# dflaxx/3d-hashjoin

Measured on AMD Instinct MI355X. Metric: probe tuples/s + build ms, exp1 key/FK |R|=1e7 |S|=1e8, 1/2/4/8 GPU, higher is better.
Workload: dtype u32; 1 GPU; exp1 key/FK plan Csr, |R|=10000000 |S|=100000000 per GPU, uniform FKs, b=1; config=B, plan=Csr, R_total=10000000, S_total=100000000, R_per_gpu=10000000, S_per_gpu=100000000, num_buckets=10000000, emit_pairs=True, parallelism=single GPU, rehearsal_one_gpu=False

## Files before the change

3d-hashjoin_amd/csrc/chain_pk.hip:

```cpp
#include <cmath>

#include "radix_seg.hpp"

namespace hj3d {
namespace {

constexpr int kPkBlock = 1024;
constexpr int kPkRounds = 8;
constexpr int kPkTile = kPkBlock * kPkRounds;
constexpr int kPkTBits = 32 - __builtin_clz(uint32_t(kPkTile - 1));
constexpr uint32_t kPkSeg = 16;
constexpr uint32_t kPkStage2 = 15872;
static_assert(kPkTile <= kPkStage2 && kPkStage2 < 65536, "the tile alone fits the stage; stage offsets in 16 bits");
constexpr uint32_t kPkMaxP1 = 2 * kPkBlock;
constexpr uint32_t kSortedMaxPk = 32;
constexpr uint32_t kOvfFlag = 0x80000000u;

enum { kCtlNovf = 0, kCtlOut = 1, kCtlTicket = 2, kCtlOvfCursor = 3, kCtlNprobe = 4, kCtlWords = 8 };


__device__ __forceinline__ void pk_ovf_append(bool me, uint2 e, uint2* __restrict__ ovf, uint64_t* ctl) {
  const uint64_t m = __ballot(me);
  if (!m) return;
  const int lane = threadIdx.x & 63;
  const int leader = __ffsll((unsigned long long)m) - 1;
  uint64_t b = 0;
  if (lane == leader) b = atomicAdd(reinterpret_cast<unsigned long long*>(ctl + kCtlNovf), (unsigned long long)__popcll(m));
  b = __shfl(b, leader, kWave);
  const uint64_t lt = lane == 0 ? 0ull : (~0ull >> (64 - lane));
  if (me) ovf[b + __popcll(m & lt)] = e;
}

template <int PPT>
struct PkPartGeom {
  static constexpr uint32_t kSeg = kPkSeg / PPT;
  static constexpr uint32_t kStage = kPkStage2;
};
template <bool IMPLICIT, bool SEL, int PPT>
__device__ __forceinline__ void pk_part_stage(const RelView& r, const PkGeom& pk, uint32_t ntiles, uint32_t cap,
                                              uint2* __restrict__ region, uint32_t* __restrict__ counts,
                                              uint2* __restrict__ ovf, uint64_t* __restrict__ ctl,
                                              const SelRange& sel, uint32_t stage_lim) {
  constexpr uint32_t SEG = PkPartGeom<PPT>::kSeg, STAGE = PkPartGeom<PPT>::kStage;
  __shared__ uint2 stage[STAGE];
  __shared__ uint32_t loc[kPkBlock * PPT];
  __shared__ uint32_t sbase[kPkBlock * PPT];
  __shared__ uint2 seginfo[STAGE / SEG];
  __shared__ uint32_t wsum[kPkBlock / kWave];
  const uint32_t me = threadIdx.x, P = pk.P, n = uint32_t(r.n);
  const int lane = threadIdx.x & 63, wid = threadIdx.x >> 6;
  const auto sl = [&](int k) __attribute__((always_inline)) { return me + uint32_t(k) * kPkBlock; };
  uint32_t my_reg[PPT];
  uint2 creg[PPT][SEG - 1];
  uint32_t my_kc[PPT], my_cur[PPT], my_end[PPT];
#pragma unroll
  for (int k = 0; k < PPT; ++k) {
    my_reg[k] = (blockIdx.x * P + sl(k)) * cap;
    my_kc[k] = 0;
    my_cur[k] = 0;
    my_end[k] = cap;
#pragma unroll
    for (int j = 0; j < int(SEG) - 1; ++j) creg[k][j] = make_uint2(0, 0);
  }
  uint32_t ha[kPkRounds], pa[SEL ? kPkRounds : 1];
  uint32_t wa[IMPLICIT ? 1 : kPkRounds];
  auto load = [&](uint32_t (&h)[kPkRounds], uint32_t (&pw)[SEL ? kPkRounds : 1],
                  uint32_t (&rw)[IMPLICIT ? 1 : kPkRounds], uint32_t tile) __attribute__((always_inline)) {
    const uint32_t base = tile * kPkTile;
#pragma unroll
    for (int j = 0; j < kPkRounds; ++j) {
      const uint32_t i = base + uint32_t(j) * kPkBlock + me;
      const char* t = r.base + uint64_t(i) * r.stride;
      h[j] = i < n ? __builtin_nontemporal_load(reinterpret_cast<const uint32_t*>(t + r.key_off)) : 0u;
      if constexpr (!IMPLICIT)
        rw[j] = i < n ? __builtin_nontemporal_load(reinterpret_cast<const uint32_t*>(t + r.row_off)) : 0u;
      if constexpr (SEL) pw[j] = i < n ? *reinterpret_cast<const uint32_t*>(t + sel.word_off) : 0u;
    }
  };
  auto to_ovf = [&](uint2 e, uint32_t p, bool me_) __attribute__((always_inline)) {
    pk_ovf_append(me_, make_uint2(pk.hash_of(e.x, p), e.y), ovf, ctl);
  };
  auto flush_carry = [&]() __attribute__((always_inline)) {
#pragma unroll
    for (int k = 0; k < PPT; ++k) {
#pragma unroll
      for (int j = 0; j < int(SEG) - 1; ++j) {
        const bool v = sl(k) < P && uint32_t(j) < my_kc[k];
        const uint32_t o = my_cur[k] + j;
        if (v && o < my_end[k]) region[my_reg[k] + o] = creg[k][j];
        to_ovf(creg[k][j], sl(k), v && o >= my_end[k]);
      }
      my_cur[k] += my_kc[k];
      my_kc[k] = 0;
    }
  };
  auto scan = [&](uint32_t v, uint32_t* total) __attribute__((always_inline)) {
    uint32_t x = v;
#pragma unroll
    for (int o = 1; o < 64; o <<= 1) {
      const uint32_t y = __shfl_up(x, o, kWave);
      if (lane >= o) x += y;
    }
    if (lane == 63) wsum[wid] = x;
    __syncthreads();
    uint32_t pre = 0, tot = 0;
#pragma unroll
    for (int w = 0; w < kPkBlock / kWave; ++w) {
      const uint32_t t = wsum[w];
      if (w < wid) pre += t;
      tot += t;
    }
    __syncthreads();
    *total = tot;
    return pre + x - v;
  };
  uint32_t npassed = 0;
  auto process = [&](uint32_t tile, uint32_t (&h)[kPkRounds], uint32_t (&pw)[SEL ? kPkRounds : 1],
                     uint32_t (&rw)[IMPLICIT ? 1 : kPkRounds]) __attribute__((always_inline)) {
    const uint32_t base = tile * kPkTile;
    uint32_t rk[kPkRounds];
#pragma unroll
    for (int j = 0; j < kPkRounds; ++j) {
      const uint32_t i = base + uint32_t(j) * kPkBlock + me;
      const uint32_t hv = murmur32(h[j]);
      const uint32_t q = pk.dnb.div(hv);
      const uint32_t bl = hv - q * pk.nb - pk.lo;
      bool pass = i < n;
      if constexpr (SEL) {
        pass = pass && sel.test(pw[j]);
        npassed += pass;
      }
      const bool ok = pass && bl < pk.nbl;
      rk[j] = kInvalid;
      if (ok) {
        const uint32_t p = pk.dw.div(bl);
        h[j] = ((bl - p * pk.W) << pk.qbits) | q;
        rk[j] = (p << kPkTBits) | atomicAdd(&loc[p], 1u);
      }
    }
    __syncthreads();
    uint32_t my_c[PPT];
#pragma unroll
    for (int k = 0; k < PPT; ++k) {
      my_c[k] = sl(k) < P ? loc[sl(k)] : 0u;
      loc[sl(k)] = 0;
    }
    const auto seg_counts = [&](int k) __attribute__((always_inline)) {
      const uint32_t L = my_kc[k] + my_c[k];
      return (L << 16) | (L / SEG);
    };
    const auto seg_sum = [&]() __attribute__((always_inline)) {
      uint32_t t = 0;
#pragma unroll
      for (int k = 0; k < PPT; ++k) t += seg_counts(k);
      return t;
// ... 404 lines not shown
                                               const uint32_t* ldir, const uint2* lent, const PkGeom& pk,
                                               uint64_t (&acc)[kProbeFields], uint2* __restrict__ out,
                                               uint64_t out_cap) {
  uint32_t nm = 0, sc = 0, nv = 0;
  constexpr int H = (K == 8 || (CK && K == 7)) ? (K + 1) / 2 : K;
#pragma unroll
  for (int g = 0; g < K; g += H) {
    uint32_t d[H], match[H], cmps[H], q[H];
    bool live[H];
#pragma unroll
    for (int j = 0; j < H && g + j < K; ++j) {
      const bool ok = (valid >> (g + j)) & 1u;
      const uint32_t x = uint32_t(v[g + j]);
      q[j] = x & pk.qmask;
      const uint32_t w = ldir[ok ? x >> pk.qbits : 0u];
      d[j] = ok ? w : 0u;
      match[j] = kInvalid;
      cmps[j] = d[j] & 0xFFFFu;
      live[j] = cmps[j] != 0 && cmps[j] <= kSortedMaxPk;
    }
#pragma unroll
    for (uint32_t c = 0; c < 3; ++c) {
      uint64_t e[H];
      bool ok[H];
#pragma unroll
      for (int j = 0; j < H && g + j < K; ++j) {
        const uint32_t nn = d[j] & 0xFFFFu;
        ok[j] = live[j] && c < nn;
        e[j] = *reinterpret_cast<const uint64_t*>(lent + (ok[j] ? (d[j] >> 16) + (c == 0 ? 0u : nn - c) : 0u));
      }
#pragma unroll
      for (int j = 0; j < H && g + j < K; ++j) asm volatile("" : "+v"(e[j]));
#pragma unroll
      for (int j = 0; j < H && g + j < K; ++j) {
        const bool hit = ok[j] && uint32_t(e[j]) == q[j];
        match[j] = hit ? uint32_t(e[j] >> 32) : match[j];
        cmps[j] = hit ? c + 1 : cmps[j];
        live[j] = live[j] && !hit;
      }
    }
#pragma unroll
    for (int j = 0; j < H && g + j < K; ++j) {
      const uint32_t nn = d[j] & 0xFFFFu, s = d[j] >> 16;
      if (live[j] && nn > 3) {
        for (uint32_t c = 3; c < nn; ++c) {
          const uint2 e = lent[s + nn - c];
          if (e.x == q[j]) {
            cmps[j] = c + 1;
            match[j] = e.y;
            break;
          }
        }
      } else if (nn > kSortedMaxPk) {
        uint32_t minrow = kInvalid, lo_m = kInvalid, hi_m = 0, cnt = 0;
        for (uint32_t k = s; k < s + nn; ++k) {
          const uint2 e = lent[k];
          minrow = min(minrow, e.y);
          if (e.x == q[j]) {
            ++cnt;
            lo_m = min(lo_m, e.y);
            hi_m = max(hi_m, e.y);
          }
        }
        if (cnt != 0 && lo_m == minrow) {
          cmps[j] = 1;
          match[j] = lo_m;
        } else if (cnt != 0) {
          uint32_t gt = 0;
          for (uint32_t k = s; k < s + nn; ++k) gt += lent[k].y > hi_m;
          cmps[j] = 2 + gt;
          match[j] = hi_m;
        }
      }
    }
#pragma unroll
    for (int j = 0; j < H && g + j < K; ++j) {
      const bool ok = (valid >> (g + j)) & 1u;
      const uint32_t row = uint32_t(v[g + j] >> 32);
      const bool m = match[j] != kInvalid;
      nv += ok;
      nm += m;
      sc += cmps[j];
      if (MODE == 1) {
        const uint64_t slot = slot0 + uint32_t((g + j) * 64);
        if (ok && slot < out_cap) pair_st(out + slot, row, match[j]);
      }
      if (CK && m) {
        acc[4] += row;
        acc[5] += match[j];
        const uint64_t ph = pair_hash(row, match[j]);
        acc[7] += ph;
        acc[8] ^= ph;
      }
    }
  }
  acc[1] += nm;
  acc[2] += nm;
  acc[3] += sc;
  (void)nv;
}

template <int MODE, bool CK>
__device__ __forceinline__ void pk_probe_hbm(uint32_t h, uint32_t row, uint32_t s, uint32_t nn,
                                             const uint2* __restrict__ ent, uint64_t slot,
                                             uint64_t (&acc)[kProbeFields], uint2* __restrict__ out,
                                             uint64_t out_cap) {
  uint32_t match = kInvalid, cmps = nn;
  if (nn <= kSortedMaxPk) {
    for (uint32_t c = 0; c < nn; ++c) {
      const uint2 e = ent[s + (c == 0 ? 0u : nn - c)];
      if (e.x == h) {
        cmps = c + 1;
        match = e.y;
        break;
      }
    }
  } else {
    uint32_t minrow = kInvalid, lo_m = kInvalid, hi_m = 0, cnt = 0;
    for (uint32_t k = s; k < s + nn; ++k) {
      const uint2 e = ent[k];
      minrow = min(minrow, e.y);
      if (e.x == h) {
        ++cnt;
        lo_m = min(lo_m, e.y);
        hi_m = max(hi_m, e.y);
      }
    }
    if (cnt != 0 && lo_m == minrow) {
      cmps = 1;
      match = lo_m;
    } else if (cnt != 0) {
      uint32_t gt = 0;
      for (uint32_t k = s; k < s + nn; ++k) gt += ent[k].y > hi_m;
      cmps = 2 + gt;
      match = hi_m;
    }
  }
  acc[3] += cmps;
  if (match != kInvalid) {
    acc[1] += 1;
    acc[2] += 1;
    if (CK) {
      acc[4] += row;
      acc[5] += match;
      const uint64_t ph = pair_hash(row, match);
      acc[7] += ph;
      acc[8] ^= ph;
    }
  }
  if (MODE == 1 && slot < out_cap)
    __builtin_nontemporal_store((uint64_t(match) << 32) | row, reinterpret_cast<uint64_t*>(out + slot));
}

__device__ __forceinline__ void pk_stage(const uint32_t* __restrict__ off, const uint2* __restrict__ ent, uint32_t b0,
                                         uint32_t nbs, uint32_t e0, uint32_t ne, const FastDiv32& dnb, uint32_t* ldir,
                                         uint2* lent) {
  constexpr int kStage = 12;
  const uint32_t nmax = max(nbs, ne);
  for (uint32_t k0 = threadIdx.x; k0 < nmax; k0 += kPkBlock * kStage) {
    uint32_t a[kStage], b[kStage];
    uint2 x[kStage];
#pragma unroll
    for (int u = 0; u < kStage; ++u) {
      const uint32_t k = k0 + u * kPkBlock;
      a[u] = k < nbs ? off[b0 + k] : 0u;
      b[u] = k < nbs ? off[b0 + k + 1] : 0u;
      x[u] = k < ne ? ent[e0 + k] : make_uint2(0, 0);
    }
#pragma unroll
    for (int u = 0; u < kStage; ++u) {
      const uint32_t k = k0 + u * kPkBlock;
      if (k < nbs) ldir[k] = ((a[u] - e0) << 16) | (b[u] - a[u]);
      if (k < ne) lent[k] = make_uint2(dnb.div(x[u].x), x[u].y);
    }
  }
}

template <int K, int MODE, bool CK>
__global__ __launch_bounds__(kPkBlock) void k_pk_probe(const uint2* __restrict__ region,
                                                       const uint32_t* __restrict__ counts, uint32_t G, uint32_t cap,
                                                       uint32_t splits, bool flat, const uint32_t* __restrict__ off,
                                                       const uint2* __restrict__ ent, PkGeom pk, FastMod fm,
                                                       uint2* __restrict__ out, uint64_t out_cap,
                                                       const uint2* __restrict__ ovf, uint64_t* __restrict__ ctl,
                                                       uint64_t* __restrict__ partials, uint64_t* __restrict__ res,
                                                       int accumulate) {
  constexpr int BLOCK = kPkBlock;
  __shared__ uint32_t lds[kLdsWords];
  __shared__ uint32_t wtot[BLOCK / kWave];
  __shared__ uint32_t rpre[BLOCK / kWave][65];
  __shared__ uint64_t bbase;
  __shared__ uint64_t red[BLOCK / kWave][kProbeFields];
  __shared__ uint32_t flag;
  const int lane = threadIdx.x & 63, wid = threadIdx.x >> 6;
  constexpr int kWaves = BLOCK / kWave;
  const uint32_t P = pk.P;
  const uint32_t p = blockIdx.x / splits, sp = blockIdx.x % splits;
  const uint32_t b0 = p * pk.W;
  const uint32_t nbs = min(pk.W, pk.nbl - b0);
  const uint32_t e0 = off[b0], e1 = off[b0 + nbs], ne = e1 - e0;
  const bool fits = (nbs + 2) + 2ull * ne <= kLdsWords;
  uint32_t* ldir = lds;
  uint2* lent = reinterpret_cast<uint2*>(lds + ((nbs + 2) & ~1u));
  uint64_t acc[kProbeFields] = {0, 0, 0, 0, 0, 0, 0, 0, 0};

  const uint32_t g_lo = uint32_t(uint64_t(G) * sp / splits), g_hi = uint32_t(uint64_t(G) * (sp + 1) / splits);
  const uint32_t nr = g_hi > g_lo + wid ? (g_hi - g_lo - wid + kWaves - 1) / kWaves : 0u;
  uint32_t my_len = 0;
  if (uint32_t(lane) < nr) my_len = counts[(g_lo + wid + kWaves * lane) * P + p];
  uint32_t wtotal;
  const uint32_t my_pre = wave_excl_scan(my_len, &wtotal);
  if (lane == 0) wtot[wid] = wtotal;
  rpre[wid][lane] = uint32_t(lane) < nr ? my_pre : ~0u;
  if (lane == 0) rpre[wid][64] = ~0u;
  __syncthreads();
  if (threadIdx.x == 0) {
    uint32_t t = 0;
    for (int w = 0; w < kWaves; ++w) t += wtot[w];
    bbase = (MODE == 1 && t) ? atomicAdd(reinterpret_cast<unsigned long long*>(ctl + kCtlOut), (unsigned long long)t) : 0ull;
  }
  uint32_t wpre = 0;
  for (int w = 0; w < wid; ++w) wpre += wtot[w];
  auto pre_at = [&](uint32_t k) __attribute__((always_inline)) { return uint32_t(__builtin_amdgcn_readlane(int(my_pre), int(k))); };
  auto len_at = [&](uint32_t k) __attribute__((always_inline)) { return uint32_t(__builtin_amdgcn_readlane(int(my_len), int(k))); };
  auto src_of = [&](uint32_t k) __attribute__((always_inline)) { return region + (g_lo + wid + kWaves * k) * P * cap + p * cap; };

  const auto src_off = [&](uint32_t k) __attribute__((always_inline)) {
    return int64_t((uint64_t(g_lo + wid + kWaves * k) * P + p) * cap);
  };
  uint32_t cr = 0, nst = rpre[wid][1];
  int64_t cbase = src_off(0);
  auto load_flat = [&](uint64_t (&v)[K], uint32_t f0) __attribute__((always_inline)) {
#pragma unroll
    for (int j = 0; j < K; ++j) {
      const uint32_t f = min(f0 + j * 64 + lane, wtotal - 1);
      while (f >= nst) {
        ++cr;
        cbase = src_off(cr) - int64_t(nst);
        nst = rpre[wid][cr + 1];
      }
      v[j] = pair_ld(region + (cbase + int64_t(f)));
    }
  };
  uint32_t r = 0, qq = 0, len = nr ? len_at(0) : 0u;
  while (r < nr && len == 0) {
    ++r;
    len = r < nr ? len_at(r) : 0u;
  }
  auto load_reg = [&](uint64_t (&v)[K], uint32_t rr, uint32_t q0, uint32_t ll) __attribute__((always_inline)) {
    const uint2* src = rr < nr ? src_of(rr) : region;
    const uint32_t last = ll ? ll - 1 : 0u;
#pragma unroll
    for (int j = 0; j < K; ++j)
      v[j] = pair_ld(src + min(q0 + j * 64 + lane, last));
  };
  auto probe_hbm_chunk = [&](const uint64_t (&v)[K], uint32_t valid, uint64_t slot0) __attribute__((always_inline)) {
#pragma unroll
    for (int j = 0; j < K; ++j) {
      if (!((valid >> j) & 1u)) continue;
      const uint32_t x = uint32_t(v[j]), bl = b0 + (x >> pk.qbits);
      const uint32_t s = off[bl];
      pk_probe_hbm<MODE, CK>(pk.hash_of(x, p), uint32_t(v[j] >> 32), s, off[bl + 1] - s, ent, slot0 + j * 64, acc,
                             out, out_cap);
    }
  };
  auto walk = [&](auto&& stage, auto&& probe) __attribute__((always_inline)) {
    constexpr uint32_t kChunk = 64 * K;
    uint64_t cur[K];
    if (flat) {
      if (wtotal) load_flat(cur, 0);
      stage();
      __syncthreads();
      if (wtotal == 0) return;
      for (uint32_t f0 = 0; f0 < wtotal; f0 += kChunk) {
        uint64_t nxt[K];
        load_flat(nxt, min(f0 + kChunk, (wtotal - 1) / kChunk * kChunk));
        uint32_t vm = 0;
#pragma unroll
        for (int j = 0; j < K; ++j) vm |= uint32_t(f0 + j * 64 + lane < wtotal) << j;
        probe(cur, vm, f0 + lane);
#pragma unroll
        for (int j = 0; j < K; ++j) cur[j] = nxt[j];
      }
    } else {
      load_reg(cur, r, qq, len);
      stage();
      __syncthreads();
      while (r < nr) {
        uint32_t nr_ = r, nq = qq + kChunk, nl = len;
        while (nr_ < nr && nq >= nl) {
          ++nr_;
          nq = 0;
          nl = nr_ < nr ? len_at(nr_) : 0u;
        }
        uint64_t nxt[K];
        load_reg(nxt, nr_, nq, nl);
        uint32_t vm = 0;
#pragma unroll
        for (int j = 0; j < K; ++j) vm |= uint32_t(qq + j * 64 + lane < len) << j;
        probe(cur, vm, pre_at(r) + qq + lane);
        r = nr_;
        qq = nq;
        len = nl;
#pragma unroll
        for (int j = 0; j < K; ++j) cur[j] = nxt[j];
      }
    }
  };
  if (fits) {
    walk([&]() __attribute__((always_inline)) { pk_stage(off, ent, b0, nbs, e0, ne, pk.dnb, ldir, lent); },
         [&](const uint64_t (&v)[K], uint32_t valid, uint32_t srel) __attribute__((always_inline)) {
           pk_probe_items<K, MODE, CK>(v, valid, bbase + wpre + srel, ldir, lent, pk, acc, out, out_cap);
         });
  } else {
    walk([&]() __attribute__((always_inline)) {},
         [&](const uint64_t (&v)[K], uint32_t valid, uint32_t srel) __attribute__((always_inline)) {
           probe_hbm_chunk(v, valid, bbase + wpre + srel);
         });
  }
  const uint64_t novf = __hip_atomic_load(ctl + kCtlNovf, __ATOMIC_RELAXED, __HIP_MEMORY_SCOPE_AGENT);
  if (novf) {
    for (;;) {
      __syncthreads();
      if (threadIdx.x == 0) {
        const uint64_t c = atomicAdd(reinterpret_cast<unsigned long long*>(ctl + kCtlOvfCursor), (unsigned long long)BLOCK);
        const uint64_t take = c < novf ? min(uint64_t(BLOCK), novf - c) : 0ull;
        bbase = c;
        flag = uint32_t(take);
        if (MODE == 1 && take)
          red[0][0] = atomicAdd(reinterpret_cast<unsigned long long*>(ctl + kCtlOut), (unsigned long long)take);
      }
      __syncthreads();
      const uint32_t take = flag;
      if (!take) break;
      const uint64_t c = bbase, ob = MODE == 1 ? red[0][0] : 0ull;
      if (threadIdx.x < take) {
        const uint2 e = ovf[c + threadIdx.x];
        const uint32_t bl = fm.mod(e.x) - pk.lo;
        const uint32_t s = off[bl];
        pk_probe_hbm<MODE, CK>(e.x, e.y, s, off[bl + 1] - s, ent, ob + threadIdx.x, acc, out, out_cap);
      }
    }
  }
  __syncthreads();
#pragma unroll
  for (int f = 1; f < kProbeFields; ++f) {
    const uint64_t w = f == kProbeFields - 1 ? wave_xor(acc[f]) : wave_sum(acc[f]);
    if (lane == 0) red[wid][f] = w;
  }
  __syncthreads();
  if (threadIdx.x < kProbeFields) {
    const int f = threadIdx.x;
    uint64_t a = 0;
    for (int w = 0; w < kWaves; ++w) a = f == kProbeFields - 1 ? (a ^ red[w][f]) : (a + red[w][f]);
    __hip_atomic_store(partials + uint64_t(blockIdx.x) * kProbeFields + f, f == 0 ? 0ull : a, __ATOMIC_RELAXED,
                       __HIP_MEMORY_SCOPE_AGENT);
  }
  if (wid == 0) {
    asm volatile("s_waitcnt vmcnt(0)" ::: "memory");
    if (threadIdx.x == 0) {
      const uint64_t t = __hip_atomic_fetch_add(ctl + kCtlTicket, 1ull, __ATOMIC_RELAXED, __HIP_MEMORY_SCOPE_AGENT);
      flag = t == gridDim.x - 1;
    }
  }
  __syncthreads();
  if (!flag) return;
  uint64_t sum[kProbeFields] = {0, 0, 0, 0, 0, 0, 0, 0, 0};
  for (uint32_t b = threadIdx.x; b < gridDim.x; b += BLOCK) {
#pragma unroll
    for (int f = 1; f < kProbeFields; ++f) {
      const uint64_t x = __hip_atomic_load(partials + uint64_t(b) * kProbeFields + f, __ATOMIC_RELAXED,
                                           __HIP_MEMORY_SCOPE_AGENT);
      sum[f] = f == kProbeFields - 1 ? (sum[f] ^ x) : (sum[f] + x);
    }
  }
  __syncthreads();
#pragma unroll
  for (int f = 1; f < kProbeFields; ++f) {
    const uint64_t w = f == kProbeFields - 1 ? wave_xor(sum[f]) : wave_sum(sum[f]);
    if (lane == 0) red[wid][f] = w;
  }
  __syncthreads();
  if (threadIdx.x < kProbeFields) {
    const int f = threadIdx.x;
    uint64_t a = 0;
    if (f == 0) {
      a = __hip_atomic_load(ctl + kCtlNprobe, __ATOMIC_RELAXED, __HIP_MEMORY_SCOPE_AGENT);
    } else {
      for (int w = 0; w < kWaves; ++w) a = f == kProbeFields - 1 ? (a ^ red[w][f]) : (a + red[w][f]);
    }
    if (accumulate) a = f == kProbeFields - 1 ? (res[f] ^ a) : (res[f] + a);
    res[f] = a;
  }
  if (!accumulate && threadIdx.x >= kProbeFields && threadIdx.x < 16) res[threadIdx.x] = 0;
  if (threadIdx.x < kCtlWords) __hip_atomic_store(ctl + threadIdx.x, 0ull, __ATOMIC_RELAXED, __HIP_MEMORY_SCOPE_AGENT);
}

constexpr uint32_t kPbW = 8192;
constexpr int kPbPer = 11;
constexpr uint32_t kPbStage = 12288;
static_assert(kPbPer * kPkBlock <= int(kPbStage), "a register-held slice fits the stage");

__global__ __launch_bounds__(256) void k_pk_slice_sums(const uint32_t* __restrict__ cnt2, uint32_t S2, uint32_t P,
                                                       uint32_t* __restrict__ tot) {
  const uint32_t p = blockIdx.x * 256 + threadIdx.x;
  if (p >= P) return;
  uint32_t t = 0;
  for (uint32_t s = 0; s < S2; ++s) t += cnt2[uint64_t(s) * P + p];
  tot[p] = t;
}

__device__ __forceinline__ void pb_lds_scan(uint32_t* a, uint32_t n, uint32_t* wsum) {
  constexpr int kPer = (kPbW + kPkBlock) / kPkBlock;
  const uint32_t t0 = threadIdx.x * kPer;
  uint32_t v[kPer], loc = 0;
#pragma unroll
  for (int k = 0; k < kPer; ++k) {
    v[k] = t0 + k < n ? a[t0 + k] : 0u;
    loc += v[k];
  }
  const int lane = threadIdx.x & 63, wid = threadIdx.x >> 6;
  uint32_t wt;
  const uint32_t pre = wave_excl_scan(loc, &wt);
  if (lane == 0) wsum[wid] = wt;
  __syncthreads();
  uint32_t base = 0;
  for (int w = 0; w < wid; ++w) base += wsum[w];
  uint32_t run = base + pre;
#pragma unroll
  for (int k = 0; k < kPer; ++k) {
    if (t0 + k < n) a[t0 + k] = run;
    run += v[k];
  }
  __syncthreads();
}

__global__ __launch_bounds__(kPkBlock) void k_pk_build(const uint2* __restrict__ fine, const uint32_t* __restrict__ cnt2,
                                                       uint32_t S2, uint32_t cap2, const uint32_t* __restrict__ ps,
                                                       PkGeom pk, uint32_t* __restrict__ off, uint2* __restrict__ ent) {
  __shared__ uint32_t cnt[kPbW + 1];
  __shared__ uint2 stage[kPbStage];
  __shared__ uint32_t wsum[kPkBlock / kWave];
  constexpr uint32_t kCap = kPbPer * kPkBlock;
  const uint32_t P = pk.P, nbl = pk.nbl, W = pk.W;
  auto gather = [&](uint32_t p, uint32_t i) __attribute__((always_inline)) {
    uint32_t run = 0;
    int64_t d = int64_t(uint64_t(p) * cap2);
    for (uint32_t sg = 0; sg < S2; ++sg) {
      if (i >= run) d = int64_t((uint64_t(sg) * P + p) * cap2) - int64_t(run);
      run += cnt2[uint64_t(sg) * P + p];
    }
    return fine[int64_t(i) + d];
  };
  const int lane = threadIdx.x & 63, wid = threadIdx.x >> 6;
  auto fits = [&](uint32_t p) __attribute__((always_inline)) {
    bool ok = true;
    for (uint32_t sg = 0; sg < S2; ++sg) ok = ok && cnt2[uint64_t(sg) * P + p] <= uint32_t(kPbPer) * 64u;
    return ok;
  };
  uint2 ea[kPbPer], eb[kPbPer];
  auto load = [&](uint2 (&e)[kPbPer], uint32_t p) __attribute__((always_inline)) {
    if (p >= P || !fits(p)) return;
    const uint32_t c = uint32_t(wid) < S2 ? cnt2[uint64_t(wid) * P + p] : 0u;
    const uint2* src = fine + (uint64_t(wid) * P + p) * cap2;
#pragma unroll
    for (int u = 0; u < kPbPer; ++u) {
      const uint32_t i = uint32_t(u) * 64u + lane;
      e[u] = i < c ? src[i] : make_uint2(0, 0);
    }
  };
  auto build = [&](uint2 (&e)[kPbPer], uint32_t p) __attribute__((always_inline)) {
    const uint32_t b0 = p * W;
    const uint32_t nbs = min(W, nbl - b0);
    const uint32_t s0 = ps[p], m = ps[p + 1] - s0;
    for (uint32_t k = threadIdx.x; k < nbs; k += kPkBlock) cnt[k] = 0;
    __syncthreads();
    if (!fits(p) || m > kCap) {
      for (uint32_t i = threadIdx.x; i < m; i += kPkBlock) atomicAdd(&cnt[gather(p, i).x >> pk.qbits], 1u);
      __syncthreads();
      pb_lds_scan(cnt, nbs, wsum);
      for (uint32_t k = threadIdx.x; k < nbs; k += kPkBlock) off[b0 + k] = s0 + cnt[k];
      if (b0 + nbs == nbl && threadIdx.x == 0) off[nbl] = s0 + m;
      __syncthreads();
      for (uint32_t i = threadIdx.x; i < m; i += kPkBlock) {
        const uint2 x = gather(p, i);
        ent[s0 + atomicAdd(&cnt[x.x >> pk.qbits], 1u)] = make_uint2(pk.hash_of(x.x, p), x.y);
      }
      __syncthreads();
      for (uint32_t k = threadIdx.x; k < nbs; k += kPkBlock) {
        const uint32_t bs = k ? cnt[k - 1] : 0u, n = cnt[k] - bs;
        if (n < 2 || n > kSortedMaxPk) continue;
        uint2* E = ent + s0 + bs;
        for (uint32_t q = 1; q < n; ++q) {
          const uint2 x = E[q];
          uint32_t j = q;
          while (j > 0 && E[j - 1].y > x.y) {
            E[j] = E[j - 1];
            --j;
          }
          E[j] = x;
        }
      }
      __syncthreads();
      return;
    }
    uint32_t rk[kPbPer];
    const uint32_t c = uint32_t(wid) < S2 ? cnt2[uint64_t(wid) * P + p] : 0u;
#pragma unroll
    for (int u = 0; u < kPbPer; ++u) {
      const bool v = uint32_t(u) * 64u + lane < c;
      const uint32_t b = v ? e[u].x >> pk.qbits : 0u;
      rk[u] = v ? (b << 16) | atomicAdd(&cnt[b], 1u) : kInvalid;
    }
    __syncthreads();
    pb_lds_scan(cnt, nbs, wsum);
    if (threadIdx.x == 0) cnt[nbs] = m;
    for (uint32_t k = threadIdx.x; k < nbs; k += kPkBlock) off[b0 + k] = s0 + cnt[k];
    if (b0 + nbs == nbl && threadIdx.x == 0) off[nbl] = s0 + m;
    __syncthreads();
#pragma unroll
    for (int u = 0; u < kPbPer; ++u)
      if (rk[u] != kInvalid) stage[cnt[rk[u] >> 16] + (rk[u] & 0xFFFFu)] = e[u];
    __syncthreads();
    for (uint32_t q = threadIdx.x; q < m; q += kPkBlock) {
      const uint2 x = stage[q];
      const uint32_t b = x.x >> pk.qbits;
      const uint32_t bs = cnt[b], n = cnt[b + 1] - bs;
      uint32_t pos = q;
      if (n >= 2 && n <= kSortedMaxPk) {
        uint32_t rr = 0;
        for (uint32_t k = bs; k < bs + n; ++k) rr += stage[k].y < x.y;
        pos = bs + rr;
      }
      ent[s0 + pos] = make_uint2(pk.hash_of(x.x, p), x.y);
    }
    __syncthreads();
  };
  load(ea, blockIdx.x);
  for (uint32_t p = blockIdx.x; p < P; p += 2 * gridDim.x) {
    load(eb, p + gridDim.x);
    build(ea, p);
    if (p + gridDim.x >= P) break;
    load(ea, p + 2 * gridDim.x);
    build(eb, p + gridDim.x);
  }
}

}

static int pk_items(double L) {
  int best = kItemsMax;
  double best_slots = 0.0;
  const double sd = std::sqrt(L > 1.0 ? L : 1.0);
  for (int K = kItemsMax; K >= kItemsMin; --K) {
    const double c = 64.0 * K;
    double slots = 0.0, wsum = 0.0;
    for (int z = -40; z <= 40; ++z) {
      const double x = L + 0.1 * z * sd, w = std::exp(-0.005 * z * z);
      slots += w * std::ceil((x < 1.0 ? 1.0 : x) / c) * c;
      wsum += w;
    }
    slots /= wsum;
    if (K == kItemsMax || slots < best_slots * 0.999) {
      best = K;
      best_slots = slots;
    }
  }
  return best;
}

bool pk_probe_applicable(const hj3d_ctx* ctx, const hj3d_table* t, uint64_t n_probe, uint32_t flags) {
  return t->desc.kind == HJ3D_CHAIN && (flags & HJ3D_PROBE_UNIQUE) && !ctx->force_direct && !ctx->pk_off &&
         n_probe >= ctx->radix_min && n_probe > 0 && t->nb_local >= 64 && t->desc.num_buckets >= 2 &&
         n_probe < (1ull << 32) && t->built;
}

static uint32_t pk_slice_width(double fill) {
  double W = double(kPkLdsWords) / (1.0 + 2.0 * fill);
  for (int i = 0; i < 6; ++i) W = (double(kPkLdsWords) - 2.0 - 12.0 * std::sqrt(W * fill)) / (1.0 + 2.0 * fill);
  return W < 64.0 ? 64u : uint32_t(W);
}

PkPlan pk_plan(const hj3d_ctx* ctx, uint32_t nbl, uint64_t n_build) {
  PkPlan pl;
  const double fill = n_build ? double(n_build) / double(nbl) : 0.0;
  uint32_t W = pk_slice_width(fill);
  if (ctx->pk_slice_max && W > ctx->pk_slice_max) W = ctx->pk_slice_max;
  if (W > nbl) W = nbl;
  uint32_t P = (nbl + W - 1) / W;
  const uint32_t ncu = uint32_t(ctx->num_cus);
  if (P >= ncu / 2) {
    uint32_t Pq = (P + ncu - 1) / ncu * ncu;
    if (P <= kPkMaxP1 && Pq > kPkMaxP1) Pq = kPkMaxP1;
    P = Pq;
    W = (nbl + P - 1) / P;
    P = (nbl + W - 1) / W;
  }
  pl.W = W;
  pl.P = P;
  pl.C = P <= kPkMaxP1 ? 1u : (P + kPkBlock - 1) / kPkBlock;
  pl.W1 = W * pl.C;
  pl.P1 = (nbl + pl.W1 - 1) / pl.W1;
  return pl;
}

static uint32_t bits(uint64_t x) {
  uint32_t b = 0;
  while (x) {
    ++b;
    x >>= 1;
  }
  return b;
}

struct PkLayout {
  uint32_t qbits = 0, ntiles = 0, G = 0, S2 = 0;
  uint64_t cap = 0, cap2 = 0, nreg = 0, nreg2 = 0;
  PkGeom pk1{}, pk{};
  uint2 *region = nullptr, *ovf = nullptr, *fine = nullptr;
  uint32_t *counts = nullptr, *fcnt = nullptr, *ps = nullptr;
  uint64_t* ctl = nullptr;
};

static hipError_t pk_layout(hj3d_ctx* ctx, const hj3d_table* t, uint64_t n, uint32_t W, uint32_t P, uint32_t C, bool two,
                            bool sums, PkLayout* L) {
  hipError_t e;
  const uint32_t nbl = t->nb_local, nb = uint32_t(t->desc.num_buckets);
  const uint32_t W1 = W * C, P1 = (nbl + W1 - 1) / W1;
  const uint32_t qbits = L->qbits = bits(0xFFFFFFFFull / nb);
  if (qbits + bits(W1 - 1) > 32) return hipErrorNotSupported;
  const uint32_t ntiles = L->ntiles = uint32_t((n + kPkTile - 1) / kPkTile);
  const uint32_t G = L->G = ntiles < uint32_t(ctx->num_cus) ? ntiles : uint32_t(ctx->num_cus);
  const uint64_t per_g = uint64_t((ntiles + G - 1) / G) * kPkTile;
  const uint64_t cap = L->cap = region_capacity(double(per_g < n ? per_g : n) / P1, kPkSeg);
  const uint64_t nreg = L->nreg = uint64_t(G) * P1;
  if (nreg * cap >= (1ull << 31)) return hipErrorNotSupported;
  const uint32_t S2 = L->S2 = two ? (G < 16u ? G : 16u) : 0u;
  const double per_gp = double(per_g < n ? per_g : n) / P;
  const uint64_t cap2 = L->cap2 = two ? region_capacity(per_gp * double((G + S2 - 1) / S2), kPkSeg) : 0;
  const uint64_t nreg2 = L->nreg2 = uint64_t(S2) * P;
  if (two && nreg2 * cap2 >= (1ull << 31)) return hipErrorNotSupported;
  if ((e = ctx->scratch[kScrPairs].ensure(nreg * cap * sizeof(uint2))) != hipSuccess) return e;
  if ((e = ctx->scratch[kScrPHist].ensure(nreg * sizeof(uint32_t))) != hipSuccess) return e;
  if ((e = ctx->scratch[kScrSortV].ensure(n * sizeof(uint2))) != hipSuccess) return e;
  if (two) {
    if ((e = ctx->scratch[kScrPk2].ensure(nreg2 * cap2 * sizeof(uint2))) != hipSuccess) return e;
    if ((e = ctx->scratch[kScrPk2Cnt].ensure(nreg2 * sizeof(uint32_t))) != hipSuccess) return e;
  }
  if (sums && (e = ctx->scratch[kScrPStart].ensure((uint64_t(P) + 1) * sizeof(uint32_t))) != hipSuccess) return e;
  if ((e = ctx->ensure_ctl()) != hipSuccess) return e;
  auto geom = [&](uint32_t w, uint32_t p) {
    PkGeom g;
    g.dnb = FastDiv32::make(nb);
    g.dw = w >= 2 ? FastDiv32::make(w) : FastDiv32{};
    g.nb = nb;
    g.lo = uint32_t(t->desc.bucket_lo);
    g.nbl = nbl;
    g.W = w;
    g.P = p;
    g.qbits = qbits;
    g.qmask = qbits >= 32 ? 0xFFFFFFFFu : ((1u << qbits) - 1);
    return g;
  };
  L->pk1 = geom(W1, P1);
  L->pk = geom(W, P);
  L->region = ctx->scratch[kScrPairs].as<uint2>();
  L->counts = ctx->scratch[kScrPHist].as<uint32_t>();
  L->ovf = ctx->scratch[kScrSortV].as<uint2>();
  L->fine = two ? ctx->scratch[kScrPk2].as<uint2>() : nullptr;
  L->fcnt = two ? ctx->scratch[kScrPk2Cnt].as<uint32_t>() : nullptr;
  L->ps = sums ? ctx->scratch[kScrPStart].as<uint32_t>() : nullptr;
  L->ctl = ctx->ctl.as<uint64_t>();
  return hipSuccess;
}

hipError_t pk_probe(hj3d_ctx* ctx, const hj3d_table* t, const hj3d_rel& r, uint32_t flags, void* out, uint64_t out_cap,
                    uint64_t* res, hipStream_t s, const SelArgs* sel) {
  hipError_t e;
  const PkPlan pl = pk_plan(ctx, t->nb_local, t->n_build);
  const bool two = pl.C > 1;
  if (pl.C > kSpMaxC) return hipErrorNotSupported;
  SelRange sr{};
  if (sel && !SelRange::from(*sel, &sr)) return hipErrorNotSupported;
  PkLayout L;
  if ((e = pk_layout(ctx, t, r.n, pl.W, pl.P, pl.C, two, false, &L)) != hipSuccess) return e;
  const uint32_t want_blocks = uint32_t(ctx->num_cus) * 2;
  const uint32_t Gp = two ? L.S2 : L.G;
  uint32_t splits = pl.P < want_blocks ? (want_blocks + pl.P - 1) / pl.P : 1u;
  if (splits > Gp) splits = Gp;
  const uint32_t nblocks = pl.P * splits;
  if ((e = ctx->scratch[kScrPartial].ensure(uint64_t(nblocks) * kProbeFields * sizeof(uint64_t))) != hipSuccess)
    return e;
  const RelView v = view_of(r);
  const bool imp = r.row_off == HJ3D_ROW_IMPLICIT;
  {
    KernelSpan tm(ctx, HJ3D_T_SCATTER);
    const uint32_t c32 = uint32_t(L.cap);
    const uint32_t slim2 = ctx->pk_stage && ctx->pk_stage < kPkStage2 ? ctx->pk_stage : kPkStage2;
#define HJ3D_PKP_LAUNCH(IMP, SEL)                                                                                   \
  if (pl.P1 > uint32_t(kPkBlock))                                                                                   \
    tm.launch(k_pk_part<IMP, SEL, 2>, dim3(L.G), dim3(kPkBlock), s, v, L.pk1, L.ntiles, c32, L.region, L.counts, L.ovf, L.ctl, sr, \
              slim2);                                                                                               \
  else                                                                                                              \
    tm.launch(k_pk_part<IMP, SEL, 1>, dim3(L.G), dim3(kPkBlock), s, v, L.pk1, L.ntiles, c32, L.region, L.counts, L.ovf, L.ctl, sr, 0u);
    if (sel) {
      if (imp) HJ3D_PKP_LAUNCH(true, true)
      else HJ3D_PKP_LAUNCH(false, true)
    } else {
      if (imp) HJ3D_PKP_LAUNCH(true, false)
      else HJ3D_PKP_LAUNCH(false, false)
    }
#undef HJ3D_PKP_LAUNCH
  }
  if ((e = hipGetLastError()) != hipSuccess) return e;
  const uint2* pregion = L.region;
  const uint32_t* pcounts = L.counts;
  uint32_t pcap = uint32_t(L.cap);
  if (two) {
    KernelSpan ts(ctx, HJ3D_T_HIST);
    ts.launch(k_pk_split, dim3(pl.P1 * L.S2), dim3(kSpBlock), s, static_cast<const uint2*>(L.region),
              static_cast<const uint32_t*>(L.counts), L.G, pl.P1, uint32_t(L.cap), L.S2, L.pk, pl.C, bits(pl.C - 1),
              uint32_t(L.cap2), L.fine, L.fcnt, L.ovf, L.ctl);
    if ((e = hipGetLastError()) != hipSuccess) return e;
    pregion = L.fine;
    pcounts = L.fcnt;
    pcap = uint32_t(L.cap2);
  }
  const bool emit = (flags & HJ3D_PROBE_EMIT) && out;
  const bool ck = flags & HJ3D_PROBE_CHECKSUM;
  const int acc = (flags & HJ3D_PROBE_ACCUMULATE) ? 1 : 0;
  const uint64_t preg = uint64_t(Gp) * pl.P;
  const bool flat = double(r.n) / double(preg) < 256.0;
// ... 107 lines not shown
```

3d-hashjoin_amd/micro/micro_slices.hip:

```cpp
#include <hip/hip_runtime.h>

#include <cstdint>
#include <cstdio>
#include <cstdlib>

#define CK(x) do { hipError_t e_ = (x); if (e_ != hipSuccess) { printf("%s:%d %s\n", __FILE__, __LINE__, hipGetErrorString(e_)); exit(1); } } while (0)

template <int BLOCK, int K, int L>
__device__ __forceinline__ void slice_walk(const uint2* __restrict__ in, const uint32_t* __restrict__ img,
                                           uint2* __restrict__ out, uint32_t per_slice, uint32_t words,
                                           uint32_t* tab, uint64_t s, bool stage, int ilv = 0, uint32_t nsl = 0) {
  constexpr uint64_t kChunk = uint64_t(BLOCK) * K;
  const uint32_t nch = (per_slice + kChunk - 1) / kChunk;
  const uint2* src = (ilv & 2) ? in : in + s * per_slice;
  uint2* dst = (ilv & 1) ? out : out + s * per_slice;
  const auto cin = [&](uint32_t c) { return (ilv & 2) ? (uint64_t(c) * nsl + s) * kChunk : uint64_t(c) * kChunk; };
  const auto cout = [&](uint32_t c) { return (ilv & 1) ? (uint64_t(c) * nsl + s) * kChunk : uint64_t(c) * kChunk; };
  uint2 cur[K], nxt[K];
  auto load = [&](uint2 (&v)[K], uint32_t ch) __attribute__((always_inline)) {
    const uint32_t cc = ch < nch ? ch : nch - 1;
    const uint64_t b = cin(cc);
    const uint32_t lim = per_slice - 1 - cc * uint32_t(kChunk);
#pragma unroll
    for (int j = 0; j < K; ++j) {
      const uint64_t i = b + min(uint32_t(j * BLOCK) + threadIdx.x, lim);
      const uint64_t x = __builtin_nontemporal_load(reinterpret_cast<const uint64_t*>(src + i));
      v[j] = make_uint2(uint32_t(x), uint32_t(x >> 32));
    }
  };
  load(cur, 0);
  const uint32_t* im = img + s * words;
  constexpr int kStage = 12;
  for (uint32_t k0 = threadIdx.x; stage && k0 < words; k0 += BLOCK * kStage) {
    uint32_t a[kStage];
#pragma unroll
    for (int u = 0; u < kStage; ++u) {
      const uint32_t k = k0 + u * BLOCK;
      a[u] = k < words ? im[k] : 0u;
    }
#pragma unroll
    for (int u = 0; u < kStage; ++u) {
      const uint32_t k = k0 + u * BLOCK;
      if (k < words) tab[k] = a[u] * 0x9E3779B1u;
    }
  }
  __syncthreads();
  for (uint32_t c = 0; c < nch; ++c) {
    load(nxt, c + 1);
    uint32_t r[K];
#pragma unroll
    for (int j = 0; j < K; ++j) r[j] = cur[j].x;
#pragma unroll
    for (int l = 0; l < L; ++l) {
#pragma unroll
      for (int j = 0; j < K; ++j) r[j] = tab[__umulhi(r[j] ^ (l * 0x85EBCA6Bu), words)] ^ cur[j].x;
    }
    const uint64_t b = cout(c);
#pragma unroll
    for (int j = 0; j < K; ++j) {
      const uint32_t i = c * uint32_t(kChunk) + uint32_t(j * BLOCK) + threadIdx.x;
      if (i < per_slice)
        __builtin_nontemporal_store((uint64_t(r[j]) << 32) | cur[j].y,
                                    reinterpret_cast<uint64_t*>(dst + b + uint32_t(j * BLOCK) + threadIdx.x));
    }
#pragma unroll
    for (int j = 0; j < K; ++j) cur[j] = nxt[j];
  }
}

template <int BLOCK, int K, int L, int MODE>
__global__ __launch_bounds__(BLOCK) void k_slice(const uint2* __restrict__ in, const uint32_t* __restrict__ img,
                                                 uint2* __restrict__ out, uint32_t per_slice, uint32_t words,
                                                 uint32_t nslices) {
  extern __shared__ uint32_t tab[];
  if (MODE == 2) {
    for (uint32_t s = blockIdx.x; s < nslices; s += gridDim.x) {
      slice_walk<BLOCK, K, L>(in, img, out, per_slice, words, tab, s, true);
      __syncthreads();
    }
  } else {
    slice_walk<BLOCK, K, L>(in, img, out, per_slice, words, tab, blockIdx.x, MODE != 1, MODE >= 3 ? MODE - 2 : 0,
                            nslices);
  }
}

template <int BLOCK, int K, int L, int MODE = 0>
void run(const char* name, const uint2* in, const uint32_t* img, uint2* out, uint64_t n, uint32_t slices,
         uint32_t words, uint32_t grid = 0) {
  auto kern = k_slice<BLOCK, K, L, MODE>;
  if (!grid) grid = slices;
  CK(hipFuncSetAttribute(reinterpret_cast<const void*>(kern), hipFuncAttributeMaxDynamicSharedMemorySize, 160 * 1024));
  hipEvent_t a, b;
  CK(hipEventCreate(&a));
  CK(hipEventCreate(&b));
  const size_t lds = size_t(words) * 4;
  const uint32_t per = uint32_t(n / slices);
  for (int w = 0; w < 3; ++w) hipLaunchKernelGGL(kern, dim3(grid), dim3(BLOCK), lds, 0, in, img, out, per, words, slices);
  CK(hipGetLastError());
  const int reps = 20;
  CK(hipEventRecord(a));
  for (int r = 0; r < reps; ++r) hipLaunchKernelGGL(kern, dim3(grid), dim3(BLOCK), lds, 0, in, img, out, per, words, slices);
  CK(hipEventRecord(b));
  CK(hipEventSynchronize(b));
  float ms;
  CK(hipEventElapsedTime(&ms, a, b));
  ms /= reps;
  printf("{\"variant\": \"%s\", \"mode\": %d, \"slices\": %u, \"block\": %d, \"lds_kb\": %.1f, \"K\": %d, \"L\": %d, \"ms\": %.4f, \"GBs\": %.0f}\n",
         name, MODE, slices, BLOCK, lds / 1024.0, K, L, ms, 16.0 * double(per) * slices / ms / 1e6);
}

template <int L>
void sweep(const uint2* in, const uint32_t* img, uint2* out, uint64_t n) {
  run<1024, 7, L>("1x1024", in, img, out, n, 1024, 37000);
  run<1024, 7, L, 1>("1x1024 nostage", in, img, out, n, 1024, 37000);
  run<1024, 7, L, 2>("1x1024 persistent", in, img, out, n, 1024, 37000, 256);
  run<1024, 7, L, 3>("1x1024 out-ilv", in, img, out, n, 1024, 37000);
  run<1024, 7, L, 4>("1x1024 in-ilv", in, img, out, n, 1024, 37000);
  run<1024, 7, L, 5>("1x1024 both-ilv", in, img, out, n, 1024, 37000);
  run<1024, 7, L>("2x1024", in, img, out, n, 2048, 18500);
  run<512, 7, L>("2x512", in, img, out, n, 2048, 18500);
  run<512, 7, L>("4x512", in, img, out, n, 4096, 9250);
  run<256, 7, L>("4x256", in, img, out, n, 4096, 9250);
}

int main() {
  const uint64_t n = 100000000ull;
  uint2 *in, *out;
  uint32_t* img;
  const uint64_t room = 110000000ull;
  CK(hipMalloc(&in, room * 8));
  CK(hipMalloc(&out, room * 8));
  CK(hipMalloc(&img, 1024ull * 37000 * 4));
  CK(hipMemset(in, 0x5A, room * 8));
  CK(hipMemset(img, 0x33, 1024ull * 37000 * 4));
  sweep<0>(in, img, out, n);
  sweep<2>(in, img, out, n);
  CK(hipFree(in));
  CK(hipFree(out));
  CK(hipFree(img));
  return 0;
}
```

Before: 121.3 billion probe tuples/s.

## Stage PK slice into LDS with 16-byte vector loads and overlap output reservation

```diff
diff --git a/3d-hashjoin_amd/csrc/chain_pk.hip b/3d-hashjoin_amd/csrc/chain_pk.hip
--- a/3d-hashjoin_amd/csrc/chain_pk.hip
+++ b/3d-hashjoin_amd/csrc/chain_pk.hip
@@ -1,6 +1,7 @@
 #include <cmath>
 
 #include "radix_seg.hpp"
+#include "pk_stage_idx.hpp"
 
 namespace hj3d {
 namespace {
@@ -711,28 +712,78 @@
     __builtin_nontemporal_store((uint64_t(match) << 32) | row, reinterpret_cast<uint64_t*>(out + slot));
 }
 
+typedef uint32_t pk_u32x4_a4 __attribute__((ext_vector_type(4), aligned(4)));
+typedef uint32_t pk_u32x2_a4 __attribute__((ext_vector_type(2), aligned(4)));
+typedef uint32_t pk_u32x4 __attribute__((ext_vector_type(4)));
+template <class Issued>
 __device__ __forceinline__ void pk_stage(const uint32_t* __restrict__ off, const uint2* __restrict__ ent, uint32_t b0,
                                          uint32_t nbs, uint32_t e0, uint32_t ne, const FastDiv32& dnb, uint32_t* ldir,
-                                         uint2* lent) {
-  constexpr int kStage = 12;
-  const uint32_t nmax = max(nbs, ne);
-  for (uint32_t k0 = threadIdx.x; k0 < nmax; k0 += kPkBlock * kStage) {
-    uint32_t a[kStage], b[kStage];
-    uint2 x[kStage];
-#pragma unroll
-    for (int u = 0; u < kStage; ++u) {
-      const uint32_t k = k0 + u * kPkBlock;
-      a[u] = k < nbs ? off[b0 + k] : 0u;
-      b[u] = k < nbs ? off[b0 + k + 1] : 0u;
-      x[u] = k < ne ? ent[e0 + k] : make_uint2(0, 0);
-    }
-#pragma unroll
-    for (int u = 0; u < kStage; ++u) {
-      const uint32_t k = k0 + u * kPkBlock;
-      if (k < nbs) ldir[k] = ((a[u] - e0) << 16) | (b[u] - a[u]);
-      if (k < ne) lent[k] = make_uint2(dnb.div(x[u].x), x[u].y);
-    }
-  }
+                                         uint2* lent, Issued&& issued) {
+  constexpr int kQ = int(kPkStageQuads), kP = int(kPkStagePairs);
+  const uint32_t t = threadIdx.x;
+  const uint32_t* o = off + b0;
+  const auto ent_at = [&](const PkStageLoad& q) __attribute__((always_inline)) {
+    return q.from_dir ? o + q.ld : reinterpret_cast<const uint32_t*>(ent + e0) + 2 * q.ld;
+  };
+  const uint32_t td = pk_stage_tail_dir(nbs);
+  const PkStageLoad qt = pk_stage_tail_ent(ne);
+  pk_u32x4 dt = *reinterpret_cast<const pk_u32x4_a4*>(o + td);
+  pk_u32x2_a4 et = *reinterpret_cast<const pk_u32x2_a4*>(ent_at(qt));
+  const uint32_t rounds = pk_stage_rounds(nbs, ne, kPkBlock);
+  const auto round = [&](uint32_t r, auto&& after_loads) __attribute__((always_inline)) {
+    pk_u32x4 dq[kQ], ex[kP];
+    uint32_t d5[kQ];
+    bool dl[kQ], el[kP];
+    uint32_t di[kQ], ei[kP];
+#pragma unroll
+    for (int u = 0; u < kQ; ++u) {
+      di[u] = pk_stage_item(r, u, t, kQ, kPkBlock);
+      const PkStageLoad q = pk_stage_quad(di[u], nbs);
+      dl[u] = q.live;
+      dq[u] = *reinterpret_cast<const pk_u32x4_a4*>(o + q.ld);
+      d5[u] = o[q.ld + 4];
+    }
+#pragma unroll
+    for (int u = 0; u < kP; ++u) {
+      ei[u] = pk_stage_item(r, u, t, kP, kPkBlock);
+      const PkStageLoad q = pk_stage_pair(ei[u], ne);
+      el[u] = q.live;
+      ex[u] = *reinterpret_cast<const pk_u32x4_a4*>(ent_at(q));
+    }
+    after_loads();
+#pragma unroll
+    for (int u = 0; u < kQ; ++u) asm volatile("" : "+v"(dq[u]), "+v"(d5[u]));
+#pragma unroll
+    for (int u = 0; u < kP; ++u) asm volatile("" : "+v"(ex[u]));
+#pragma unroll
+    for (int u = 0; u < kQ; ++u) {
+      pk_u32x4 w;
+      w.x = pk_dir_word(dq[u].x, dq[u].y, e0);
+      w.y = pk_dir_word(dq[u].y, dq[u].z, e0);
+      w.z = pk_dir_word(dq[u].z, dq[u].w, e0);
+      w.w = pk_dir_word(dq[u].w, d5[u], e0);
+      if (dl[u]) *reinterpret_cast<pk_u32x4*>(ldir + 4 * di[u]) = w;
+    }
+#pragma unroll
+    for (int u = 0; u < kP; ++u) {
+      pk_u32x4 w = ex[u];
+      w.x = dnb.div(w.x);
+      w.z = dnb.div(w.z);
+      if (el[u]) *reinterpret_cast<pk_u32x4*>(lent + 2 * ei[u]) = w;
+    }
+  };
+  round(0, [&]() __attribute__((always_inline)) {
+    __builtin_amdgcn_sched_barrier(0);
+    issued();
+    __builtin_amdgcn_sched_barrier(0);
+  });
+  for (uint32_t r = 1; r < rounds; ++r) round(r, []() {});
+  asm volatile("" : "+v"(dt), "+v"(et));
+  if (t < kPkStageTailDir) {
+    const uint32_t a = t == 0 ? dt.x : t == 1 ? dt.y : dt.z, b = t == 0 ? dt.y : t == 1 ? dt.z : dt.w;
+    ldir[td + t] = pk_dir_word(a, b, e0);
+  }
+  if (t == 0 && qt.live) lent[qt.ld] = make_uint2(dnb.div(et.x), et.y);
 }
 
 template <int K, int MODE, bool CK>
@@ -745,7 +796,7 @@
                                                        uint64_t* __restrict__ partials, uint64_t* __restrict__ res,
                                                        int accumulate) {
   constexpr int BLOCK = kPkBlock;
-  __shared__ uint32_t lds[kLdsWords];
+  __shared__ __attribute__((aligned(16))) uint32_t lds[kLdsWords];
   __shared__ uint32_t wtot[BLOCK / kWave];
   __shared__ uint32_t rpre[BLOCK / kWave][65];
   __shared__ uint64_t bbase;
@@ -757,27 +808,35 @@
   const uint32_t p = blockIdx.x / splits, sp = blockIdx.x % splits;
   const uint32_t b0 = p * pk.W;
   const uint32_t nbs = min(pk.W, pk.nbl - b0);
-  const uint32_t e0 = off[b0], e1 = off[b0 + nbs], ne = e1 - e0;
-  const bool fits = (nbs + 2) + 2ull * ne <= kLdsWords;
-  uint32_t* ldir = lds;
-  uint2* lent = reinterpret_cast<uint2*>(lds + ((nbs + 2) & ~1u));
   uint64_t acc[kProbeFields] = {0, 0, 0, 0, 0, 0, 0, 0, 0};
 
   const uint32_t g_lo = uint32_t(uint64_t(G) * sp / splits), g_hi = uint32_t(uint64_t(G) * (sp + 1) / splits);
   const uint32_t nr = g_hi > g_lo + wid ? (g_hi - g_lo - wid + kWaves - 1) / kWaves : 0u;
-  uint32_t my_len = 0;
-  if (uint32_t(lane) < nr) my_len = counts[(g_lo + wid + kWaves * lane) * P + p];
+  uint32_t vz;
+  asm volatile("v_mov_b32 %0, 0" : "=v"(vz));
+  const uint32_t lr = nr ? min(uint32_t(lane), nr - 1) : 0u;
+  uint32_t my_len = counts[(nr ? g_lo + wid + kWaves * lr : 0u) * P + p];
+  uint32_t ve0 = off[b0 + vz], ve1 = off[b0 + nbs + vz];
+  asm volatile("" : "+v"(my_len), "+v"(ve0), "+v"(ve1));
+  my_len = uint32_t(lane) < nr ? my_len : 0u;
+  const uint32_t e0 = __builtin_amdgcn_readfirstlane(ve0), ne = __builtin_amdgcn_readfirstlane(ve1) - e0;
+  const bool fits = pk_slice_staged(nbs, ne, kLdsWords);
+  uint32_t* ldir = lds;
+  uint2* lent = reinterpret_cast<uint2*>(lds + pk_lent_word(nbs));
   uint32_t wtotal;
   const uint32_t my_pre = wave_excl_scan(my_len, &wtotal);
   if (lane == 0) wtot[wid] = wtotal;
   rpre[wid][lane] = uint32_t(lane) < nr ? my_pre : ~0u;
   if (lane == 0) rpre[wid][64] = ~0u;
   __syncthreads();
-  if (threadIdx.x == 0) {
-    uint32_t t = 0;
-    for (int w = 0; w < kWaves; ++w) t += wtot[w];
-    bbase = (MODE == 1 && t) ? atomicAdd(reinterpret_cast<unsigned long long*>(ctl + kCtlOut), (unsigned long long)t) : 0ull;
-  }
+  uint64_t my_base = 0;
+  auto reserve = [&]() __attribute__((always_inline)) {
+    if (MODE == 1 && threadIdx.x == 0) {
+      uint32_t t = 0;
+      for (int w = 0; w < kWaves; ++w) t += wtot[w];
+      if (t) my_base = atomicAdd(reinterpret_cast<unsigned long long*>(ctl + kCtlOut), (unsigned long long)t);
+    }
+  };
   uint32_t wpre = 0;
   for (int w = 0; w < wid; ++w) wpre += wtot[w];
   auto pre_at = [&](uint32_t k) __attribute__((always_inline)) { return uint32_t(__builtin_amdgcn_readlane(int(my_pre), int(k))); };
@@ -829,6 +888,7 @@
     if (flat) {
       if (wtotal) load_flat(cur, 0);
       stage();
+      if (threadIdx.x == 0) bbase = my_base;
       __syncthreads();
       if (wtotal == 0) return;
       for (uint32_t f0 = 0; f0 < wtotal; f0 += kChunk) {
@@ -844,6 +904,7 @@
     } else {
       load_reg(cur, r, qq, len);
       stage();
+      if (threadIdx.x == 0) bbase = my_base;
       __syncthreads();
       while (r < nr) {
         uint32_t nr_ = r, nq = qq + kChunk, nl = len;
@@ -867,12 +928,12 @@
     }
   };
   if (fits) {
-    walk([&]() __attribute__((always_inline)) { pk_stage(off, ent, b0, nbs, e0, ne, pk.dnb, ldir, lent); },
+    walk([&]() __attribute__((always_inline)) { pk_stage(off, ent, b0, nbs, e0, ne, pk.dnb, ldir, lent, reserve); },
          [&](const uint64_t (&v)[K], uint32_t valid, uint32_t srel) __attribute__((always_inline)) {
            pk_probe_items<K, MODE, CK>(v, valid, bbase + wpre + srel, ldir, lent, pk, acc, out, out_cap);
          });
   } else {
-    walk([&]() __attribute__((always_inline)) {},
+    walk([&]() __attribute__((always_inline)) { reserve(); },
          [&](const uint64_t (&v)[K], uint32_t valid, uint32_t srel) __attribute__((always_inline)) {
            probe_hbm_chunk(v, valid, bbase + wpre + srel);
          });
@@ -1136,7 +1197,7 @@
 
 static uint32_t pk_slice_width(double fill) {
   double W = double(kPkLdsWords) / (1.0 + 2.0 * fill);
-  for (int i = 0; i < 6; ++i) W = (double(kPkLdsWords) - 2.0 - 12.0 * std::sqrt(W * fill)) / (1.0 + 2.0 * fill);
+  for (int i = 0; i < 6; ++i) W = (double(kPkLdsWords) - 3.0 - 12.0 * std::sqrt(W * fill)) / (1.0 + 2.0 * fill);
   return W < 64.0 ? 64u : uint32_t(W);
 }
 
diff --git a/3d-hashjoin_amd/csrc/pk_stage_idx.hpp b/3d-hashjoin_amd/csrc/pk_stage_idx.hpp
--- /dev/null
+++ b/3d-hashjoin_amd/csrc/pk_stage_idx.hpp
@@ -0,0 +1,51 @@
+#pragma once
+
+#include <stdint.h>
+
+#if defined(__HIPCC__)
+#define HJ3D_PK_HD __host__ __device__ inline __attribute__((always_inline))
+#else
+#define HJ3D_PK_HD inline
+#endif
+
+namespace hj3d {
+
+constexpr uint32_t kPkStageQuads = 3;
+constexpr uint32_t kPkStagePairs = 6;
+
+HJ3D_PK_HD uint32_t pk_lent_word(uint32_t nbs) { return (nbs + 3u) & ~3u; }
+HJ3D_PK_HD bool pk_slice_fits(uint32_t nbs, uint32_t ne, uint32_t lds_words) {
+  return uint64_t(pk_lent_word(nbs)) + 2ull * ne <= lds_words;
+}
+HJ3D_PK_HD bool pk_slice_staged(uint32_t nbs, uint32_t ne, uint32_t lds_words) {
+  return nbs >= 4 && pk_slice_fits(nbs, ne, lds_words);
+}
+HJ3D_PK_HD uint32_t pk_stage_rounds(uint32_t nbs, uint32_t ne, uint32_t block) {
+  const uint32_t per = block * 4u * kPkStageQuads;
+  const uint32_t n = nbs > ne ? nbs : ne;
+  return n / per + (n % per != 0);
+}
+HJ3D_PK_HD uint32_t pk_stage_item(uint32_t r, uint32_t u, uint32_t t, uint32_t per, uint32_t block) {
+  return (r * per + u) * block + t;
+}
+
+struct PkStageLoad {
+  uint32_t ld;
+  bool live;
+  bool from_dir;
+};
+HJ3D_PK_HD PkStageLoad pk_stage_quad(uint32_t i, uint32_t nbs) {
+  const bool live = i < nbs / 4u;
+  return {live ? 4u * i : nbs - 4u, live, false};
+}
+HJ3D_PK_HD PkStageLoad pk_stage_pair(uint32_t i, uint32_t ne) {
+  const bool live = i < ne / 2u;
+  return {live ? 2u * i : ne >= 2u ? ne - 2u : 0u, live, ne < 2u};
+}
+constexpr uint32_t kPkStageTailDir = 3;
+HJ3D_PK_HD uint32_t pk_stage_tail_dir(uint32_t nbs) { return nbs - 3u; }
+HJ3D_PK_HD PkStageLoad pk_stage_tail_ent(uint32_t ne) { return {ne ? ne - 1u : 0u, ne != 0u, ne == 0u}; }
+
+HJ3D_PK_HD uint32_t pk_dir_word(uint32_t a, uint32_t b, uint32_t e0) { return ((a - e0) << 16) | (b - a); }
+
+}
diff --git a/3d-hashjoin_amd/micro/micro_slices.hip b/3d-hashjoin_amd/micro/micro_slices.hip
--- a/3d-hashjoin_amd/micro/micro_slices.hip
+++ b/3d-hashjoin_amd/micro/micro_slices.hip
@@ -9,7 +9,7 @@
 template <int BLOCK, int K, int L>
 __device__ __forceinline__ void slice_walk(const uint2* __restrict__ in, const uint32_t* __restrict__ img,
                                            uint2* __restrict__ out, uint32_t per_slice, uint32_t words,
-                                           uint32_t* tab, uint64_t s, bool stage, int ilv = 0, uint32_t nsl = 0) {
+                                           uint32_t* tab, uint64_t s, int stage, int ilv = 0, uint32_t nsl = 0) {
   constexpr uint64_t kChunk = uint64_t(BLOCK) * K;
   const uint32_t nch = (per_slice + kChunk - 1) / kChunk;
   const uint2* src = (ilv & 2) ? in : in + s * per_slice;
@@ -31,7 +31,7 @@
   load(cur, 0);
   const uint32_t* im = img + s * words;
   constexpr int kStage = 12;
-  for (uint32_t k0 = threadIdx.x; stage && k0 < words; k0 += BLOCK * kStage) {
+  for (uint32_t k0 = threadIdx.x; stage == 1 && k0 < words; k0 += BLOCK * kStage) {
     uint32_t a[kStage];
 #pragma unroll
     for (int u = 0; u < kStage; ++u) {
@@ -42,6 +42,22 @@
     for (int u = 0; u < kStage; ++u) {
       const uint32_t k = k0 + u * BLOCK;
       if (k < words) tab[k] = a[u] * 0x9E3779B1u;
+    }
+  }
+  constexpr int kWide = 10;
+  const uint32_t quads = words / 4;
+  for (uint32_t k0 = threadIdx.x; stage == 2 && k0 < quads; k0 += BLOCK * kWide) {
+    typedef uint32_t u32x4 __attribute__((ext_vector_type(4)));
+    u32x4 a[kWide];
+#pragma unroll
+    for (int u = 0; u < kWide; ++u)
+      a[u] = reinterpret_cast<const u32x4*>(im)[min(k0 + u * BLOCK, quads - 1)];
+#pragma unroll
+    for (int u = 0; u < kWide; ++u) asm volatile("" : "+v"(a[u]));
+#pragma unroll
+    for (int u = 0; u < kWide; ++u) {
+      const uint32_t k = k0 + u * BLOCK;
+      if (k < quads) reinterpret_cast<u32x4*>(tab)[k] = a[u] * 0x9E3779B1u;
     }
   }
   __syncthreads();
@@ -72,15 +88,15 @@
 __global__ __launch_bounds__(BLOCK) void k_slice(const uint2* __restrict__ in, const uint32_t* __restrict__ img,
                                                  uint2* __restrict__ out, uint32_t per_slice, uint32_t words,
                                                  uint32_t nslices) {
-  extern __shared__ uint32_t tab[];
+  extern __shared__ __attribute__((aligned(16))) uint32_t tab[];
   if (MODE == 2) {
     for (uint32_t s = blockIdx.x; s < nslices; s += gridDim.x) {
-      slice_walk<BLOCK, K, L>(in, img, out, per_slice, words, tab, s, true);
+      slice_walk<BLOCK, K, L>(in, img, out, per_slice, words, tab, s, 1);
       __syncthreads();
     }
   } else {
-    slice_walk<BLOCK, K, L>(in, img, out, per_slice, words, tab, blockIdx.x, MODE != 1, MODE >= 3 ? MODE - 2 : 0,
-                            nslices);
+    slice_walk<BLOCK, K, L>(in, img, out, per_slice, words, tab, blockIdx.x, MODE == 1 ? 0 : MODE == 6 ? 2 : 1,
+                            MODE >= 3 && MODE <= 5 ? MODE - 2 : 0, nslices);
   }
 }
 
@@ -112,6 +128,7 @@
 template <int L>
 void sweep(const uint2* in, const uint32_t* img, uint2* out, uint64_t n) {
   run<1024, 7, L>("1x1024", in, img, out, n, 1024, 37000);
+  run<1024, 7, L, 6>("1x1024 stage16", in, img, out, n, 1024, 37000);
   run<1024, 7, L, 1>("1x1024 nostage", in, img, out, n, 1024, 37000);
   run<1024, 7, L, 2>("1x1024 persistent", in, img, out, n, 1024, 37000, 256);
   run<1024, 7, L, 3>("1x1024 out-ilv", in, img, out, n, 1024, 37000);
```

Result: no change. 121.4 billion probe tuples/s (median of 3 runs) (+0.1%).
